# JunkyByte/deepcharuco

Measured on AMD Instinct MI355X. Metric: frames/sec end-to-end (detect+refine) at 320x240; corner-id match vs ref, higher is better.
Workload: dtype f32; 1 GPU; bs=32/GPU x1 GPU(s) = 32 frames of 320x240, full detect+refine pipeline (BASELINE configs[1]); preset=cfg2, batch_per_gpu=32, global_batch=32, height=240, width=320, corner_pool_per_gpu=2048, frames=board, truncated_frames=0, distinct_ids_in_batch=16, parallelism=frames sharded, 1 process/GPU x1

## Files before the change

deepcharuco_amd/_lib.py:

```python
from __future__ import annotations

import ctypes as C
import os
import subprocess
from typing import Optional

_HERE = os.path.dirname(os.path.abspath(__file__))
LIB_PATH = os.environ.get("DCX_LIB") or os.path.join(_HERE, "libdeepcharuco_amd.so")
CSRC = os.path.join(_HERE, "csrc")

_lib: Optional[C.CDLL] = None


class DcxError(RuntimeError):
    def __init__(self, code: int, where: str):
        self.code = code
        try:
            msg = lib().dcx_error_string(code).decode()
        except Exception:
            msg = "?"
        super().__init__(f"{where} failed with code {code}: {msg}")


def build(force: bool = False, verbose: bool = False) -> str:
# ... 3 lines not shown
    res = subprocess.run(cmd, capture_output=True, text=True)
    if res.returncode != 0:
        raise RuntimeError("building libdeepcharuco_amd.so failed:\n" + res.stdout[-4000:] + res.stderr[-8000:])
    if verbose:
        print(res.stdout)
    return LIB_PATH


_vp, _i, _l, _sz = C.c_void_p, C.c_int, C.c_long, C.c_size_t

SIGNATURES = {
    "dcx_version": (C.c_char_p, []),
    "dcx_error_string": (C.c_char_p, [_i]),
    "dcx_detector_create": (_i, [C.POINTER(_vp), C.POINTER(_vp), _i, _i]),
    "dcx_detector_destroy": (_i, [_vp]),
    "dcx_refiner_create": (_i, [C.POINTER(_vp), C.POINTER(_vp), _i]),
    "dcx_refiner_destroy": (_i, [_vp]),
    "dcx_detector_workspace_bytes": (_sz, [_vp, _i, _i, _i]),
    "dcx_refiner_workspace_bytes": (_sz, [_vp, _i]),
    "dcx_bgr2gray": (_i, [_vp, _l, _i, _i, _i, _i, _vp, _vp]),
    "dcx_bgr2gray_legacy14": (_i, [_vp, _l, _i, _i, _i, _i, _vp, _vp]),
    "dcx_pre_image": (_i, [_vp, _vp, _sz, _vp]),
    "dcx_detector_forward": (_i, [_vp, _vp, _l, _i, _vp, _i, _i, _i, _vp, _sz, _vp, _vp, _vp]),
    "dcx_detector_decode": (_i, [_vp, _i, _i, _i, _vp, _i, _i, _vp, _vp, _vp, _vp, _vp]),
    "dcx_pred_to_keypoints": (_i, [_vp, _vp, _i, _i, _i, _i, _i, _i, _i, _vp, _vp, _vp, _vp, _vp]),
    "dcx_label_to_keypoints": (_i, [_vp, _vp, _i, _i, _i, _i, _i, _vp, _vp, _vp, _vp, _vp]),
    "dcx_build_patch_table": (_i, [_vp, _vp, _i, _i, _vp, _vp, _vp]),
    "dcx_extract_patches_u8": (_i, [_vp, _l, _i, _i, _i, _vp, _vp, _i, _vp, _vp]),
    "dcx_extract_patches_f32": (_i, [_vp, _i, _i, _vp, _vp, _i, _vp, _vp]),
    "dcx_refiner_forward": (_i, [_vp, _vp, _i, _vp, _vp, _vp, _sz, _vp, _vp, _vp, _vp]),
    "dcx_argmax2d": (_i, [_vp, _i, _i, _i, _vp, _vp]),
    "dcx_pipeline_workspace_bytes": (_sz, [_vp, _vp, _i, _i, _i, _i]),
    "dcx_infer_batch": (_i, [_vp, _vp, _vp, _l, _i, _i, _i, _i, _i, _i, _i, _vp, _sz, _vp, _vp, _vp, _vp, _vp, _vp]),
    "dcx_stream_synchronize": (_i, [_vp]),
    "dcx_solve_pnp_pool": (_i, [_vp, _vp, _vp, _vp, _i, _i, _i, _i, C.c_double, C.POINTER(C.c_double), C.POINTER(C.c_double), _i,
                               _vp, _vp, _vp]),
    "dcx_solve_pnp_ransac_workspace_bytes": (_sz, [_i, _i, _i]),
    "dcx_solve_pnp_ransac_pool": (_i, [_vp, _vp, _vp, _vp, _i, _i, _i, _i, C.c_double, C.POINTER(C.c_double), C.POINTER(C.c_double), _i,
                                      _i, C.c_double, _i, C.c_uint, _vp, _sz, _vp, _vp, _vp, _vp, _vp]),
    "dcx_calibrate_workspace_bytes": (_sz, [_i]),
    "dcx_calibrate_pool": (_i, [_vp, _vp, _vp, _vp, _i, _i, _i, _i, C.c_double, _i, _i, _vp, _sz, _vp, _vp,
                               C.POINTER(C.c_double), _vp]),
    "dcx_calibrate_ransac_workspace_bytes": (_sz, [_i, _i, _i]),
    "dcx_calibrate_ransac_pool": (_i, [_vp, _vp, _vp, _vp, _i, _i, _i, _i, C.c_double, _i, _i, _i, C.c_double, C.c_double, _i, _i,
                                      C.c_uint, _vp, _sz, _vp, _vp, _vp, _vp, C.POINTER(C.c_double), _vp]),
    "dcx_stereo_calibrate_workspace_bytes": (_sz, [_i, _i, _i]),
    "dcx_stereo_calibrate_pool": (_i, [_vp] * 10 + [_i, _i, _i, _i, _i, C.c_double, C.POINTER(C.c_double), C.POINTER(C.c_double), _i,
                                      C.POINTER(C.c_double), C.POINTER(C.c_double), _i, _vp, _sz, _vp, _vp, _vp,
                                      C.POINTER(C.c_double), _vp]),
    "dcx_undistort_rectify_map": (_i, [C.POINTER(C.c_double), C.POINTER(C.c_double), _i, C.POINTER(C.c_double),
                                      C.POINTER(C.c_double), _i, _i, _vp, _vp]),
    "dcx_rectify_points_pool": (_i, [_vp, _vp, _i, C.POINTER(C.c_double), C.POINTER(C.c_double), _i, C.POINTER(C.c_double),
                                    C.POINTER(C.c_double), _vp, _vp]),
    "dcx_remap_u8": (_i, [_vp, _l, _i, _i, _i, _i, _vp, _i, _i, _i, _i, _vp, _vp]),
    "dcx_sgm_workspace_bytes": (_sz, [_i, _i, _i, _i]),
    "dcx_sgm_u8": (_i, [_vp, _l, _i, _vp, _l, _i, _i, _i, _i, _i, _i, _i, _i, _i, _i, _vp, _vp, _sz, _vp]),
    "dcx_sgm_u8_paths": (_i, [_vp, _l, _i, _vp, _l, _i, _i, _i, _i, _i, _i, _i, _i, _i, _i, _i, _vp, _vp, _sz, _vp]),
    "dcx_disparity_to_points": (_i, [_vp, _i, _i, _i, _i, C.POINTER(C.c_double), _vp, _vp]),
    "dcx_filter_speckles_workspace_bytes": (_sz, [_i, _i, _i]),
    "dcx_filter_speckles_s16": (_i, [_vp, _vp, _i, _i, _i, _i, _i, _i, _vp, _sz, _vp]),
    "dcx_conv_layer": (_i, [_vp, _i, _i, _i, _i, _vp, _vp, _vp, _vp, _vp, _vp, _i, _i, _i, _i, _i, _i, _vp, _vp]),
    "dcx_nchw_to_c4": (_i, [_vp, _i, _i, _i, _i, _vp, _vp]),
    "dcx_c4_to_nchw": (_i, [_vp, _i, _i, _i, _i, _vp, _vp]),
    "dcx_set_timing": (_i, [_i]),
    "dcx_get_timing": (_i, []),
    "dcx_profile_enabled": (_i, []),
# ... 63 lines not shown
```

deepcharuco_amd/csrc/dcx_api.hip:

```cpp
#include "dcx_common.h"

#include <math.h>
#include <stdlib.h>
#include <string.h>
#include <new>
#include <vector>

namespace {

constexpr float kBnEps = 1e-5f;

inline size_t align_up(size_t v, size_t a) { return (v + a - 1) / a * a; }


std::vector<float> pack_conv(const float* w, int cout, int cin, int ks, int cout_pad) {
    const int taps = ks * ks, cq = cin / 4;
    std::vector<float> out((size_t)taps * cq * cout_pad * 4, 0.0f);
    for (int o = 0; o < cout; ++o)
        for (int i = 0; i < cin; ++i)
            for (int t = 0; t < taps; ++t)
                out[(((size_t)t * cq + (i >> 2)) * cout_pad + o) * 4 + (i & 3)] = w[((size_t)o * cin + i) * taps + t];
    return out;
}

// ... 269 lines not shown
        std::vector<float> w(2 * wsz), b(512), g(512), be(512), mu(512), var(512);
        memcpy(w.data(), pa.w, wsz * 4); memcpy(w.data() + wsz, da.w, wsz * 4);
        auto cat = [](std::vector<float>& dst, const float* x, const float* y) {
            memcpy(dst.data(), x, 256 * 4); memcpy(dst.data() + 256, y, 256 * 4);
        };
        cat(b, pa.b, da.b); cat(g, pa.g, da.g); cat(be, pa.be, da.be); cat(mu, pa.mu, da.mu); cat(var, pa.var, da.var);
        rc = make_layer(HostConv{w.data(), b.data(), g.data(), be.data(), mu.data(), var.data()}, 128, 512, 3,
                        &d->heads_a);
    }
    if (rc == 0) rc = make_layer(hc(54, false), 256, 65, 1, &d->head_loc);
    if (rc == 0) rc = make_layer(hc(62, false), 256, n_ids + 1, 1, &d->head_ids);
    if (rc != 0) { dcx_detector_destroy(d); return rc; }
    *out = d;
    return 0;
}

extern "C" int dcx_detector_destroy(dcx_detector* d) {
    if (!d) return 0;
    free_layer(d->first);
    for (auto& l : d->enc) free_layer(l);
    free_layer(d->heads_a); free_layer(d->head_loc); free_layer(d->head_ids);
    delete d;
    return 0;
}

extern "C" size_t dcx_detector_workspace_bytes(const dcx_detector* det, int batch, int height, int width) {
    if (!det || batch <= 0 || height <= 0 || width <= 0) return 0;
    return det_layout(det->n_ids, batch, height, width).total;
}

namespace {
int detector_run(const dcx_detector* det, const uint8_t* d_frames_u8, long frame_stride, int pitch, int pix,
                 const float* d_images_f32, int batch, int height, int width, void* d_ws, size_t ws_bytes,
                 bool with_heads, float* d_loc_nchw, float* d_ids_nchw, int32_t* zero_words, int n_zero, void* stream);
}

extern "C" int dcx_detector_forward(const dcx_detector* det, const uint8_t* d_frames_u8, long frame_stride, int pitch,
                                    const float* d_images_f32, int batch, int height, int width, void* d_ws,
                                    size_t ws_bytes, float* d_loc_nchw, float* d_ids_nchw, void* stream) {
    return detector_run(det, d_frames_u8, frame_stride, pitch, DCX_PIX_GRAY8, d_images_f32, batch, height, width, d_ws, ws_bytes, true,
                        d_loc_nchw, d_ids_nchw, nullptr, 0, stream);
}

namespace {
int detector_run(const dcx_detector* det, const uint8_t* d_frames_u8, long frame_stride, int pitch, int pix,
                 const float* d_images_f32, int batch, int height, int width, void* d_ws, size_t ws_bytes,
                 bool with_heads, float* d_loc_nchw, float* d_ids_nchw, int32_t* zero_words, int n_zero, void* stream) {
    if (!det || !d_ws) return DCX_E_ARG;
    if ((d_frames_u8 == nullptr) == (d_images_f32 == nullptr)) return DCX_E_ARG;
    if (batch <= 0 || height < 8 || width < 8) return DCX_E_SHAPE;
    const DetWs L = det_layout(det->n_ids, batch, height, width);
    if (ws_bytes < L.total) return DCX_E_WS;
    hipStream_t s = (hipStream_t)stream;
    char* ws = (char*)d_ws;
    float* buf0 = (float*)(ws + L.buf0);
    float* buf1 = (float*)(ws + L.buf1);
    float* loc = (float*)(ws + L.loc);
    float* ids = (float*)(ws + L.ids);
    const int h = height, w = width;
    int rc;
    const int pt0 = dcx_prof_begin(DCX_PROF_CONV1A, batch, s);
    if (d_frames_u8)
        rc = dcx_launch_conv1_u8(d_frames_u8, frame_stride, pitch, pix, batch, h, w, 1, det->first.w, det->first.bias,
                                 det->first.alpha, det->first.beta, buf0, nullptr, zero_words, n_zero, s);
    else
        rc = dcx_launch_conv1_f32(d_images_f32, (long)h * w, w, batch, h, w, 1, det->first.w, det->first.bias,
                                  det->first.alpha, det->first.beta, buf0, nullptr, s);
    if (rc) return rc;
    if ((rc = dcx_prof_end(pt0, s))) return rc;
    struct Step { int layer, div, pool; };
    static const Step steps[7] = {{0, 1, 1}, {1, 2, 0}, {2, 2, 1}, {3, 4, 0}, {4, 4, 1}, {5, 8, 0}, {6, 8, 0}};
    float* src = buf0;
    float* dst = buf1;
    for (const Step& st : steps) {
        const DevLayer& l = det->enc[st.layer];
        DcxConvArgs a = conv_args(l, src, batch, l.cin / 4, 0, h / st.div, w / st.div, 0, 1, dst, l.cout / 4, nullptr);
        rc = dcx_launch_conv_mfma(a, 3, st.pool, DCX_EPI_BNRELU, s);
        if (rc) return rc;
        float* t = src; src = dst; dst = t;
    }
    const int hc = h / 8, wc = w / 8;
    {
        DcxConvArgs a = conv_args(det->heads_a, src, batch, 32, 0, hc, wc, 0, 1, dst, 128, nullptr);
        rc = dcx_launch_conv_mfma(a, 3, 0, DCX_EPI_BNRELU, s);
        if (rc) return rc;
    }
    if (!with_heads) return 0;
    {
        DcxConvArgs a = conv_args(det->head_loc, dst, batch, 128, 0, 1, hc * wc, 0, 0, loc, 17, nullptr);
        rc = dcx_launch_conv_mfma(a, 1, 0, DCX_EPI_RAW, s);
        if (rc) return rc;
    }
    {
        DcxConvArgs a = conv_args(det->head_ids, dst, batch, 128, 64, 1, hc * wc, 0, 0, ids, L.ids_quads, nullptr);
        rc = dcx_launch_conv_mfma(a, 1, 0, DCX_EPI_RAW, s);
        if (rc) return rc;
    }
    if (d_loc_nchw) { rc = dcx_c4_to_nchw(loc, batch, 65, hc, wc, d_loc_nchw, stream); if (rc) return rc; }
    if (d_ids_nchw) { rc = dcx_c4_to_nchw(ids, batch, det->n_ids + 1, hc, wc, d_ids_nchw, stream); if (rc) return rc; }
    return 0;
}
}

extern "C" int dcx_detector_decode(const dcx_detector* det, int batch, int height, int width, void* d_ws,
                                   int dust_bin, int kmax, int32_t* d_counts, int32_t* d_rows, int32_t* d_loc_argmax,
                                   int32_t* d_ids_argmax, void* stream) {
    if (!det || !d_ws) return DCX_E_ARG;
    if (batch <= 0 || height < 8 || width < 8) return DCX_E_SHAPE;
    const DetWs L = det_layout(det->n_ids, batch, height, width);
    const int hc = height / 8, wc = width / 8;
    const long cells = (long)hc * wc;
    char* ws = (char*)d_ws;
// ... 91 lines not shown
        {7, 16, 1, 1, 0},
        {8, 32, 0, 1, 0},
    };
    float* src = buf0;
    float* dst = buf1;
    for (const Step& st : steps) {
        const DevLayer& l = rf->mid[st.layer];
        DcxConvArgs a = conv_args(l, src, p, l.cin / 4, 0, st.hin, st.hin, st.ups, st.pad, dst, l.cout / 4, lim);
        a.n_hint = lim != nullptr ? n_hint : 0;
        rc = dcx_launch_conv_mfma(a, 3, st.pool, DCX_EPI_BNRELU, s);
        if (rc) return rc;
        float* t = src; src = dst; dst = t;
    }
    int heat_tiles = 0;
    {
        DcxConvArgs a = conv_args(rf->head_a, src, p, 16, 0, 32, 32, 1, 1, nullptr, 16, lim);
        a.head_w = rf->head_w; a.head_b = rf->head_b; a.heat = d_heat;
        a.part_val = (float*)(ws + L.pval); a.part_idx = (int*)(ws + L.pidx);
        heat_tiles = dcx_conv_heat_tiles(a.ho, a.wo, a.w_ups2w != nullptr ? 1 : 0);
        if (heat_tiles <= 0 || heat_tiles > kRefTiles) return DCX_E_SHAPE;
        rc = dcx_launch_conv_mfma(a, 3, 0, DCX_EPI_HEAT, s);
        if (rc) return rc;
    }
    const int pt1 = dcx_prof_begin(DCX_PROF_FINALIZE, p, s);
    rc = dcx_launch_refine_finalize((const float*)(ws + L.pval), (const int*)(ws + L.pidx), heat_tiles, 64, p, lim,
                                    d_table, d_corners, d_xy, s);
    if (rc) return rc;
    return dcx_prof_end(pt1, s);
}
}

namespace {
struct PipeWs { size_t det, table, ctrl, ref, total; int ctrl_words; };
PipeWs pipe_layout(const dcx_detector* det, const dcx_refiner* rf, int b, int h, int w, int pool) {
    PipeWs L;
    size_t off = 0;
    L.det = off; off = align_up(off + det_layout(det->n_ids, b, h, w).total, 256);
    L.table = off; off = align_up(off + (size_t)pool * 16, 256);
    L.ctrl_words = 64 + b;
    L.ctrl = off; off = align_up(off + (size_t)L.ctrl_words * 4, 256);
    L.ref = off; off = align_up(off + (rf ? ref_layout(pool).total : 0), 256);
    L.total = off;
    return L;
}
}

extern "C" size_t dcx_pipeline_workspace_bytes(const dcx_detector* det, const dcx_refiner* rf, int batch, int height,
                                               int width, int pool) {
    if (!det || batch <= 0 || height <= 0 || width <= 0 || pool <= 0) return 0;
    return pipe_layout(det, rf, batch, height, width, pool).total;
}

namespace {
int infer_range(const dcx_detector* det, const dcx_refiner* rf, const uint8_t* d_frames_u8, long frame_stride, int pitch, int pix,
                int batch, int height, int width, int dust_bin, int pool, char* ws, size_t ws_bytes, int32_t* d_counts,
                int32_t* d_starts, int32_t* d_rows, float* d_xy, float* d_conf, hipStream_t s, bool timing) {
    void* stream = (void*)s;
    const PipeWs L = pipe_layout(det, rf, batch, height, width, pool);
    if (ws_bytes < L.total) return DCX_E_WS;
    int rc = timing ? timing_mark(0, s) : 0;
    if (rc) return rc;
    int32_t* ctrl = (int32_t*)(ws + L.ctrl);
    rc = detector_run(det, d_frames_u8, frame_stride, pitch, pix, nullptr, batch, height, width, ws + L.det, L.table - L.det,
                      false, nullptr, nullptr, ctrl, L.ctrl_words, stream);
    if (rc) return rc;
    if (timing && (rc = timing_mark(1, s))) return rc;
    int32_t* table = (int32_t*)(ws + L.table);
    {
        const DetWs D = det_layout(det->n_ids, batch, height, width);
        const int hc = height / 8, wc = width / 8;
        const float* act = (const float*)(ws + L.det + D.buf0);
        int32_t* codes = (int32_t*)(ws + L.det + D.codes);
        DcxPoolOut po;
        po.tickets = ctrl + 64; po.cursor = ctrl; po.counts = d_counts; po.starts = d_starts; po.rows = d_rows;
        po.table = rf ? table : nullptr; po.conf = d_conf; po.conf_cells = (float*)(ws + L.det + D.conf);
        po.wc = wc; po.pool = pool;
        const int pt = dcx_prof_begin(DCX_PROF_TAIL, batch, s);
        rc = dcx_launch_tail(act, batch, hc * wc, det->head_loc.w, det->head_loc.bias, det->head_ids.w, det->head_ids.bias,
                             det->head_ids.cout_pad, det->n_ids + 1, dust_bin, codes, nullptr, nullptr, &po, s);
        if (rc) return rc;
        if ((rc = dcx_prof_end(pt, s))) return rc;
    }
    if (timing && (rc = timing_mark(2, s))) return rc;
    if (rf == nullptr) return timing ? timing_mark(3, s) : 0;
    const long expect = (long)batch * det->n_ids;
    const FrameSrc src{d_frames_u8, frame_stride, pitch, pix, height, width};
    rc = refiner_run(rf, nullptr, &src, pool, (int)(expect < pool ? expect : pool), ctrl, table,
                     ws + L.ref, L.total - L.ref, nullptr, d_xy, nullptr, stream);
    if (rc) return rc;
    return timing ? timing_mark(3, s) : 0;
}
}

extern "C" int dcx_infer_batch(const dcx_detector* det, const dcx_refiner* rf, const uint8_t* d_frames_u8,
                               long frame_stride, int pitch, int pixel_format, int batch, int height, int width, int dust_bin,
                               int pool, void* d_ws, size_t ws_bytes, int32_t* d_counts, int32_t* d_starts, int32_t* d_rows,
                               float* d_xy, float* d_conf, void* stream) {
    if (!det || !d_frames_u8 || !d_ws || !d_counts || !d_starts || !d_rows) return DCX_E_ARG;
    if (rf != nullptr && d_xy == nullptr) return DCX_E_ARG;
    if (pixel_format != DCX_PIX_GRAY8 && pixel_format != DCX_PIX_BGR8 && pixel_format != DCX_PIX_BGR8_LEGACY14) return DCX_E_ARG;
    if (pool <= 0 || pool > (1 << 22)) return DCX_E_SHAPE;
    if (batch <= 0 || batch > (1 << 20) || height < 8 || width < 8) return DCX_E_SHAPE;
    if (pitch < width * (pixel_format == DCX_PIX_GRAY8 ? 1 : 3)) return DCX_E_SHAPE;
    if (dust_bin < 0 || dust_bin > 255) return DCX_E_NIDS;
    hipStream_t s = (hipStream_t)stream;
    char* ws = (char*)d_ws;
    return infer_range(det, rf, d_frames_u8, frame_stride, pitch, pixel_format, batch, height, width, dust_bin, pool, ws, ws_bytes,
                       d_counts, d_starts, d_rows, d_xy, d_conf, s, true);
}

extern "C" int dcx_stream_synchronize(void* stream) { return (int)hipStreamSynchronize((hipStream_t)stream); }

extern "C" int dcx_set_timing(int enabled) { g_timing = enabled != 0; return 0; }
extern "C" int dcx_get_timing(void) { return g_timing ? 1 : 0; }

extern "C" int dcx_last_timings(float* h_ms4) {
    if (!h_ms4) return DCX_E_ARG;
    if (!g_ev_ok) return DCX_E_ARG;
    DCX_CHECK_HIP(hipEventElapsedTime(&h_ms4[0], g_ev[0], g_ev[1]));
    DCX_CHECK_HIP(hipEventElapsedTime(&h_ms4[1], g_ev[1], g_ev[2]));
    DCX_CHECK_HIP(hipEventElapsedTime(&h_ms4[2], g_ev[2], g_ev[3]));
    DCX_CHECK_HIP(hipEventElapsedTime(&h_ms4[3], g_ev[0], g_ev[3]));
    return 0;
}

extern "C" int dcx_conv_layer(const float* d_in, int n, int cin, int hin, int win, const float* h_w, const float* h_b,
                              const float* h_g, const float* h_be, const float* h_mu, const float* h_var, int cout,
                              int ksize, int pad, int ups, int pool, int relu, float* d_out, void* stream) {
    if (!d_in || !h_w || !h_b || !d_out) return DCX_E_ARG;
    if (cin % 32 != 0 || (ksize != 3 && ksize != 1) || n <= 0) return DCX_E_SHAPE;
    const bool bn = h_g != nullptr;
    if (bn != (relu != 0)) return DCX_E_ARG;
    if (bn && (!h_be || !h_mu || !h_var)) return DCX_E_ARG;
    if (const int rc = dcx_xcd_init()) return rc;
    DevLayer l;
    int rc = make_layer(HostConv{h_w, h_b, h_g, h_be, h_mu, h_var}, cin, cout, ksize, &l, ups != 0);
    if (rc) return rc;
    DcxConvArgs a;
    if (ksize == 1) {
        if (pad != 0 || ups != 0 || pool != 0) { free_layer(l); return DCX_E_SHAPE; }
        a = conv_args(l, d_in, n, cin / 4, 0, 1, hin * win, 0, 0, d_out, (cout + 3) / 4, nullptr);
// ... 10 lines not shown
```

deepcharuco_amd/inference.py:

```python
from __future__ import annotations

import ctypes as _ctypes
import warnings
from typing import List, Optional

import numpy as np
import torch

from . import _lib
from .imgproc import _opencv, bgr2gray
from .models._handles import require_cuda, unwrap
from .models.model_utils import extract_patches, pre_bgr_image, pred_to_keypoints
from .models.net import dcModel, lModel
from .models.refinenet import RefineNet, lRefineNet
from .pnp import (solve_pnp_batch_device, solve_pnp_device, solve_pnp_host, solve_pnp_pool, solve_pnp_ransac_batch_device,
                  solve_pnp_ransac_device, solve_pnp_ransac_host, solve_pnp_ransac_pool, unpack_poses, unpack_ransac)

__all__ = ["load_models", "infer_image", "infer_image_staged", "infer_batch", "infer_batch_device", "unpack_results", "packed_len",
           "solve_pnp", "solve_pnp_batch", "solve_pnp_submit", "set_deterministic", "InferenceModel", "calibrate_xcd",
           "set_xcd_weights", "get_xcd_weights", "solve_pnp_host", "solve_pnp_device", "solve_pnp_batch_device", "solve_pnp_pool",
           "unpack_poses", "solve_pnp_ransac_host", "solve_pnp_ransac_device", "solve_pnp_ransac_batch_device",
           "solve_pnp_ransac_pool", "unpack_ransac"]

DEFAULT_KMAX = 64
# ... 83 lines not shown
    with torch.cuda.device(dev):
        torch.cuda.synchronize()
        _lib.check(_lib.lib().dcx_calibrate_xcd(int(rounds), w, _lib.current_stream()), "dcx_calibrate_xcd")
    from .graph import clear_graph_cache
    clear_graph_cache()
    return [float(v) for v in w]


def set_xcd_weights(weights=None, device="cuda") -> None:
    dev = require_cuda(device)
    arr = None if weights is None else (_ctypes.c_float * 8)(*[float(v) for v in weights])
    with torch.cuda.device(dev):
        _lib.check(_lib.lib().dcx_set_xcd_weights(arr), "dcx_set_xcd_weights")
    from .graph import clear_graph_cache
    clear_graph_cache()


def get_xcd_weights(device="cuda") -> List[float]:
    dev = require_cuda(device)
    w = (_ctypes.c_float * 8)()
    with torch.cuda.device(dev):
        _lib.check(_lib.lib().dcx_get_xcd_weights(w), "dcx_get_xcd_weights")
    return [float(v) for v in w]


PIXEL_FORMATS = {"gray": 0, "opencv4": 1, "legacy14": 2}


def packed_len(batch: int, pool: int, conf: bool = False) -> int:
    return 2 * batch + (8 if conf else 6) * pool


def launch_pipeline(det, ref, frames_ptr: int, b: int, h: int, w: int, bpp: int, pix: int, dust_bin_ids: int, pool: int,
                    ws: torch.Tensor, out_ptr: int, conf: bool = False) -> None:
    counts_p, starts_p, rows_p = out_ptr, out_ptr + 4 * b, out_ptr + 8 * b
    xy_p = rows_p + 16 * pool
    conf_p = xy_p + 8 * pool
    _lib.check(_lib.lib().dcx_infer_batch(det.handle, ref.handle if ref else None, frames_ptr, h * w * bpp, w * bpp, pix, b, h, w,
                                          dust_bin_ids, pool, ws.data_ptr(), ws.numel(), counts_p, starts_p, rows_p,
                                          xy_p if ref else None, conf_p if conf else None, _lib.current_stream()), "dcx_infer_batch")


def infer_batch_device(frames: torch.Tensor, dust_bin_ids: int, deepc, refinenet=None, kmax: int = DEFAULT_KMAX,
                       out: Optional[torch.Tensor] = None, ws: Optional[torch.Tensor] = None, pool: Optional[int] = None,
                       conf: bool = False, bgr_variant: str = "opencv4") -> torch.Tensor:
    det, ref = unwrap(deepc), unwrap(refinenet)
    dev = det.device
    if (not isinstance(frames, torch.Tensor) or frames.device != dev or frames.dtype != torch.uint8 or not frames.is_contiguous()
            or not (frames.ndim == 3 or (frames.ndim == 4 and frames.shape[3] == 3))):
        raise ValueError("frames must be a contiguous (B,H,W) gray or (B,H,W,3) BGR uint8 tensor on the model's GPU")
    b, h, w = frames.shape[:3]
    bpp = 1 if frames.ndim == 3 else 3
    if bgr_variant not in ("opencv4", "legacy14"):
        raise ValueError(f"unknown BGR->gray variant {bgr_variant!r}")
    pix = PIXEL_FORMATS["gray" if bpp == 1 else bgr_variant]
    if pool is None:
        pool = b * kmax
    if pool <= 0:
        raise ValueError("pool must be positive")
    L = _lib.lib()
    with torch.cuda.device(dev):
        nbytes = L.dcx_pipeline_workspace_bytes(det.handle, ref.handle if ref else None, b, h, w, pool)
        if nbytes == 0:
            raise ValueError("bad batch/shape for dcx_pipeline_workspace_bytes")
        if ws is None:
            ws = det._ws.get("pipe", dev, nbytes)
        elif ws.device != dev or ws.dtype != torch.uint8 or not ws.is_contiguous() or ws.numel() < nbytes:
            raise ValueError(f"ws must be a contiguous uint8 tensor of >= {nbytes} bytes on {dev}")
        n_i32 = packed_len(b, pool, conf)
        if out is None:
            out = torch.empty((n_i32,), dtype=torch.int32, device=dev)
        elif out.device != dev or out.dtype != torch.int32 or out.numel() != n_i32 or not out.is_contiguous():
            raise ValueError(f"out must be a contiguous int32 tensor of {n_i32} elements on {dev}")
        launch_pipeline(det, ref, frames.data_ptr(), b, h, w, bpp, pix, dust_bin_ids, pool, ws, out.data_ptr(), conf)
    return out


def unpack_results(packed: np.ndarray, batch: int, pool: int, refined: bool, conf: bool = False):
    packed = np.asarray(packed, dtype=np.int32)
    counts = packed[:batch]
    head = packed[:2 * batch].tolist()
    rows = packed[2 * batch:2 * batch + 4 * pool].reshape(pool, 4)
    xy = packed[2 * batch + 4 * pool:2 * batch + 6 * pool].view(np.float32).reshape(pool, 2)
    cf = packed[2 * batch + 6 * pool:2 * batch + 8 * pool].view(np.float32).reshape(pool, 2) if conf else None
    res: List[Optional[np.ndarray]] = []
    confs: List[Optional[np.ndarray]] = []
    for b in range(batch):
        k, s0 = head[b], head[batch + b]
        if k == 0:
            res.append(np.array([]))
            confs.append(np.zeros((0, 2), np.float32))
            continue
        if s0 + k > pool:
            res.append(None)
            confs.append(None)
            continue
        rb = rows[s0:s0 + k]
        order = rb[:, 2].argsort(kind="stable")
        a = np.empty((k, 3), np.float64 if refined else np.int64)
        a[:, 0:2] = xy[s0:s0 + k] if refined else rb[:, 0:2]
        a[:, 2] = rb[:, 2]
# ... 143 lines not shown
```

deepcharuco_amd/stream.py:

```python
from __future__ import annotations

import time
import warnings
from typing import Iterable, Iterator, List, Optional, Tuple

import numpy as np
import torch

from .inference import DEFAULT_KMAX, infer_batch, infer_batch_device, packed_len, solve_pnp_submit, unpack_results
from .models._handles import unwrap
from .pnp import (POSE_WORDS, ransac_workspace_bytes, solve_pnp_batch_device, solve_pnp_pool, solve_pnp_ransac_batch_device,
                  solve_pnp_ransac_pool, unpack_poses, unpack_ransac)


class FrameStream:
    def __init__(self, dust_bin_ids: int, deepc, refinenet=None, batch: int = 32, height: int = 240,
                 width: int = 320, kmax: int = DEFAULT_KMAX, depth: int = 2, pnp: Optional[dict] = None,
                 compute_streams: int = 1, bgr: bool = False, h2d_on_compute: Optional[bool] = None, pnp_device: bool = False,
                 pnp_ransac: Optional[dict] = None):
        det = unwrap(deepc)
        self.dev = det.device
        self.dust_bin_ids, self.deepc, self.refinenet = dust_bin_ids, deepc, refinenet
        self.batch, self.h, self.w, self.kmax, self.depth = batch, height, width, kmax, depth
        self.pool = batch * kmax
        self.bgr = bool(bgr)
        self.h2d_on_compute = compute_streams > 1 if h2d_on_compute is None else bool(h2d_on_compute)
        self.pnp = pnp
        self.pnp_device = bool(pnp_device) and pnp is not None
        if pnp_ransac is not None and not self.pnp_device:
            raise ValueError("pnp_ransac needs pnp=... and pnp_device=True")
        self.pnp_ransac = None if pnp_ransac is None else dict(pnp_ransac)
        if not (1 <= compute_streams <= depth):
            raise ValueError("compute_streams must be between 1 and depth")
        n_out = packed_len(batch, self.pool)
        shape = (batch, height, width, 3) if self.bgr else (batch, height, width)
        with torch.cuda.device(self.dev):
            self.copy_stream = torch.cuda.Stream()
            self.compute = [torch.cuda.Stream() for _ in range(compute_streams)] if compute_streams > 1 else None
            self.pin_in = [torch.empty(shape, dtype=torch.uint8).pin_memory() for _ in range(depth)]
            self.dev_in = [torch.empty(shape, dtype=torch.uint8, device=self.dev) for _ in range(depth)]
            self.dev_out = [torch.empty((n_out,), dtype=torch.int32, device=self.dev) for _ in range(depth)]
            self.pin_out = [torch.empty((n_out,), dtype=torch.int32).pin_memory() for _ in range(depth)]
# ... 84 lines not shown
        return retired

    def _resolve(self, r):
        return r if len(r) == 2 or self.pnp_device else (r[0], r[1], [f.result() for f in r[2]])

    def flush(self) -> Iterator[Tuple]:
        order = sorted((p[0], s) for s, p in enumerate(self._pending) if p is not None)
        for _, slot in order:
            yield self._resolve(self._collect(slot))

    def run(self, batches: Iterable[np.ndarray]) -> Iterator[Tuple]:
        if self.pnp is None:
            for fr in batches:
                r = self.submit(fr)
                if r is not None:
                    yield r
            yield from self.flush()
            return
        held = None
        for fr in batches:
            r = self.submit(fr)
            if held is not None:
                yield self._resolve(held)
                held = None
            if r is not None:
                held = r
        if held is not None:
            yield self._resolve(held)
        yield from self.flush()


class ResidentStream:

    def __init__(self, dust_bin_ids: int, deepc, refinenet=None, batch: int = 32, height: int = 240, width: int = 320,
                 kmax: int = DEFAULT_KMAX, compute_streams: int = 1, depth: Optional[int] = None, bgr: bool = False,
                 raw: bool = False, timing: bool = False):
        det = unwrap(deepc)
        self.dev = det.device
        self.dust_bin_ids, self.deepc, self.refinenet = dust_bin_ids, deepc, refinenet
        self.batch, self.h, self.w, self.kmax = batch, height, width, kmax
        self.pool = batch * kmax
        self.bgr, self.raw, self.timing = bool(bgr), bool(raw), bool(timing)
        if compute_streams < 1:
            raise ValueError("compute_streams must be >= 1")
        self.depth = depth = compute_streams + 2 if depth is None else depth
        if depth < compute_streams:
            raise ValueError("depth must be >= compute_streams")
        n_out = packed_len(batch, self.pool)
        with torch.cuda.device(self.dev):
            self.compute = [torch.cuda.Stream() for _ in range(compute_streams)]
            self.dev_out = [torch.empty((n_out,), dtype=torch.int32, device=self.dev) for _ in range(depth)]
            self.pin_out = [torch.empty((n_out,), dtype=torch.int32).pin_memory() for _ in range(depth)]
            self.ev_in = [torch.cuda.Event() for _ in range(depth)]
            self.ev_start = [torch.cuda.Event(enable_timing=True) for _ in range(depth)] if self.timing else None
            self.ev_done = [torch.cuda.Event(enable_timing=self.timing) for _ in range(depth)]
        self._pending: List[Optional[Tuple[int, torch.Tensor, torch.cuda.Stream]]] = [None] * depth
        self._ticket = 0
        self.gpu_ms: List[float] = []
        self.host_enqueue_s = 0.0
        self.host_wait_s = 0.0

    def reset_stats(self) -> None:
        self.gpu_ms = []
        self.host_enqueue_s = self.host_wait_s = 0.0

    def _collect(self, slot: int):
        ticket, frames, compute = self._pending[slot]
        self._pending[slot] = None
        n = frames.shape[0]
        t0 = time.perf_counter()
        self.ev_done[slot].synchronize()
        self.host_wait_s += time.perf_counter() - t0
        if self.timing:
            self.gpu_ms.append(self.ev_start[slot].elapsed_time(self.ev_done[slot]))
        packed = self.pin_out[slot].numpy()[:packed_len(n, self.pool)]
        need = int(packed[:n].astype(np.int64).sum())
        if need > self.pool:
            warnings.warn(f"a batch produced {need} corners > pool={self.pool} (batch x kmax); re-running it with pool={need}")
            n_big = packed_len(n, need)
            with torch.cuda.device(self.dev):
                host = torch.empty((n_big,), dtype=torch.int32).pin_memory()
                done = torch.cuda.Event()
                with torch.cuda.stream(compute):
                    big = infer_batch_device(frames, self.dust_bin_ids, self.deepc, self.refinenet, pool=need)
                    host.copy_(big, non_blocking=True)
                    done.record(compute)
            t0 = time.perf_counter()
            done.synchronize()
            self.host_wait_s += time.perf_counter() - t0
            packed = host.numpy()
            if self.raw:
                return ticket, packed
            return ticket, unpack_results(packed, n, need, self.refinenet is not None)[0]
        if self.raw:
            return ticket, packed.copy()
        return ticket, unpack_results(packed, n, self.pool, self.refinenet is not None)[0]

    def submit(self, frames: torch.Tensor):
        want = (self.h, self.w, 3) if self.bgr else (self.h, self.w)
        if (not isinstance(frames, torch.Tensor) or frames.device != self.dev or frames.dtype != torch.uint8
                or not frames.is_contiguous() or tuple(frames.shape[1:]) != want or not (1 <= frames.shape[0] <= self.batch)):
            raise ValueError(f"frames must be a contiguous (1 <= n <= batch, {', '.join(map(str, want))}) uint8 tensor on {self.dev}")
        n = frames.shape[0]
        slot = self._ticket % self.depth
        retired = self._collect(slot) if self._pending[slot] is not None else None
        t0 = time.perf_counter()
        n_out = packed_len(n, self.pool)
        with torch.cuda.device(self.dev):
            compute = self.compute[self._ticket % len(self.compute)]
            self.ev_in[slot].record(torch.cuda.current_stream())
            with torch.cuda.stream(compute):
                compute.wait_event(self.ev_in[slot])
                if self.timing:
                    self.ev_start[slot].record(compute)
                infer_batch_device(frames, self.dust_bin_ids, self.deepc, self.refinenet, out=self.dev_out[slot][:n_out],
                                   pool=self.pool)
                self.pin_out[slot][:n_out].copy_(self.dev_out[slot][:n_out], non_blocking=True)
                self.ev_done[slot].record(compute)
        self._pending[slot] = (self._ticket, frames, compute)
        self._ticket += 1
        self.host_enqueue_s += time.perf_counter() - t0
        return retired

    def flush(self) -> Iterator[Tuple]:
        order = sorted((p[0], s) for s, p in enumerate(self._pending) if p is not None)
        for _, slot in order:
            yield self._collect(slot)

    def run(self, batches: Iterable[torch.Tensor]) -> Iterator[Tuple]:
        for fr in batches:
            r = self.submit(fr)
            if r is not None:
                yield r
        yield from self.flush()
```

include/deepcharuco_amd.h:

```cpp
#ifndef DEEPCHARUCO_AMD_H
#define DEEPCHARUCO_AMD_H

#include <stddef.h>
#include <stdint.h>

#ifdef __cplusplus
extern "C" {
#endif

#define DCX_E_ARG      (-1)
#define DCX_E_SHAPE    (-2)
#define DCX_E_WS       (-3)
#define DCX_E_NIDS     (-4)

typedef struct dcx_detector dcx_detector;
typedef struct dcx_refiner  dcx_refiner;

const char* dcx_version(void);
const char* dcx_error_string(int code);

int dcx_detector_create(dcx_detector** out, const float* const* h_tensors, int n_tensors, int n_ids);
int dcx_detector_destroy(dcx_detector* det);
int dcx_refiner_create(dcx_refiner** out, const float* const* h_tensors, int n_tensors);
int dcx_refiner_destroy(dcx_refiner* rf);
// ... 24 lines not shown
                          int dust_bin, int kmax,
                          int32_t* d_counts, int32_t* d_rows,
                          int32_t* d_loc_argmax, int32_t* d_ids_argmax, void* stream);
int dcx_label_to_keypoints(const long long* d_loc, const long long* d_ids, int batch, int hc, int wc, int dust_bin, int kmax,
                           int32_t* d_counts, int32_t* d_rows, int32_t* d_codes, int32_t* d_bad, void* stream);

int dcx_build_patch_table(const int32_t* d_counts, const int32_t* d_rows, int batch, int kmax,
                          int32_t* d_table, int32_t* d_total, void* stream);

int dcx_extract_patches_u8(const uint8_t* d_frames, long frame_stride, int pitch, int height, int width,
                           const int32_t* d_table, const int32_t* d_total, int max_patches,
                           float* d_patches, void* stream);
int dcx_extract_patches_f32(const float* d_images, int height, int width,
                            const int32_t* d_table, const int32_t* d_total, int max_patches,
                            float* d_patches, void* stream);

int dcx_refiner_forward(const dcx_refiner* rf, const float* d_patches, int max_patches,
                        const int32_t* d_total, const int32_t* d_table,
                        void* d_ws, size_t ws_bytes,
                        int32_t* d_corners, float* d_xy, float* d_heat, void* stream);

int dcx_argmax2d(const float* d_x, int k, int h, int w, int32_t* d_out, void* stream);

#define DCX_PIX_GRAY8          0
#define DCX_PIX_BGR8           1
#define DCX_PIX_BGR8_LEGACY14  2
size_t dcx_pipeline_workspace_bytes(const dcx_detector* det, const dcx_refiner* rf,
                                    int batch, int height, int width, int pool);
int dcx_infer_batch(const dcx_detector* det, const dcx_refiner* rf,
                    const uint8_t* d_frames_u8, long frame_stride, int pitch, int pixel_format,
                    int batch, int height, int width, int dust_bin, int pool,
                    void* d_ws, size_t ws_bytes,
                    int32_t* d_counts, int32_t* d_starts, int32_t* d_rows, float* d_xy, float* d_conf, void* stream);
int dcx_stream_synchronize(void* stream);

#define DCX_PNP_OK          0
#define DCX_PNP_TOO_FEW     1
#define DCX_PNP_TRUNCATED   2
#define DCX_PNP_BAD_ID      3
#define DCX_PNP_DEGENERATE  4
#define DCX_PNP_NONFINITE   5
int dcx_solve_pnp_pool(const int32_t* d_counts, const int32_t* d_starts, const int32_t* d_rows,
                       const float* d_xy , int batch, int pool,
                       int col_count, int row_count, double square_len,
                       const double* h_camera9, const double* h_dist, int n_dist,
                       int32_t* d_status, double* d_pose ,
                       void* stream);

#define DCX_PNP_NO_CONSENSUS 6
size_t dcx_solve_pnp_ransac_workspace_bytes(int batch, int pool, int iterations);
int dcx_solve_pnp_ransac_pool(const int32_t* d_counts, const int32_t* d_starts, const int32_t* d_rows,
                              const float* d_xy , int batch, int pool,
                              int col_count, int row_count, double square_len,
                              const double* h_camera9, const double* h_dist, int n_dist,
                              int iterations, double reproj_error, int min_inliers, unsigned seed,
                              void* d_workspace, size_t workspace_bytes,
                              int32_t* d_status, double* d_pose , int32_t* d_info ,
                              uint8_t* d_inliers , void* stream);

#define DCX_CALIB_OK          0
#define DCX_CALIB_NO_VIEWS    1
#define DCX_CALIB_DEGENERATE  2
#define DCX_CALIB_NONFINITE   3
size_t dcx_calibrate_workspace_bytes(int batch);
int dcx_calibrate_pool(const int32_t* d_counts, const int32_t* d_starts, const int32_t* d_rows,
                       const float* d_xy , int batch, int pool,
// ... 98 lines not shown
```

Before: 10240 frames/s.

## Prefetch conv1a on a side stream to overlap with previous batch's tail

Splits the first detector conv (conv1a from u8 frames) into a separate entry point that writes into a double-buffered front workspace on a side stream. The main compute stream waits on that event and runs the rest of the pipeline from the prefetched activation, recording a detector-done event so the next front launch can reuse the buffer safely. This lets conv1a of batch N+1 overlap with decode/refine of batch N. The pipeline also now writes results straight into pinned host memory, dropping the device output buffer and the device-to-host copy. The cost is two extra full-resolution 64-channel activation buffers plus the added cross-stream event synchronisation.

```diff
diff --git a/deepcharuco_amd/_lib.py b/deepcharuco_amd/_lib.py
--- a/deepcharuco_amd/_lib.py
+++ b/deepcharuco_amd/_lib.py
@@ -59,6 +59,10 @@
     "dcx_argmax2d": (_i, [_vp, _i, _i, _i, _vp, _vp]),
     "dcx_pipeline_workspace_bytes": (_sz, [_vp, _vp, _i, _i, _i, _i]),
     "dcx_infer_batch": (_i, [_vp, _vp, _vp, _l, _i, _i, _i, _i, _i, _i, _i, _vp, _sz, _vp, _vp, _vp, _vp, _vp, _vp]),
+    "dcx_front_bytes": (_sz, [_vp, _i, _i, _i]),
+    "dcx_detector_front": (_i, [_vp, _vp, _l, _i, _i, _i, _i, _i, _vp, _sz, _vp]),
+    "dcx_infer_batch_prefetched": (_i, [_vp, _vp, _vp, _l, _i, _i, _i, _i, _i, _i, _i, _vp, _sz, _vp, _sz, _vp, _vp, _vp, _vp, _vp,
+                                       _vp, _vp]),
     "dcx_stream_synchronize": (_i, [_vp]),
     "dcx_solve_pnp_pool": (_i, [_vp, _vp, _vp, _vp, _i, _i, _i, _i, C.c_double, C.POINTER(C.c_double), C.POINTER(C.c_double), _i,
                                _vp, _vp, _vp]),
diff --git a/deepcharuco_amd/csrc/dcx_api.hip b/deepcharuco_amd/csrc/dcx_api.hip
--- a/deepcharuco_amd/csrc/dcx_api.hip
+++ b/deepcharuco_amd/csrc/dcx_api.hip
@@ -325,20 +325,36 @@
 namespace {
 int detector_run(const dcx_detector* det, const uint8_t* d_frames_u8, long frame_stride, int pitch, int pix,
                  const float* d_images_f32, int batch, int height, int width, void* d_ws, size_t ws_bytes,
-                 bool with_heads, float* d_loc_nchw, float* d_ids_nchw, int32_t* zero_words, int n_zero, void* stream);
+                 bool with_heads, float* d_loc_nchw, float* d_ids_nchw, int32_t* zero_words, int n_zero, const float* act0,
+                 void* stream);
 }
 
 extern "C" int dcx_detector_forward(const dcx_detector* det, const uint8_t* d_frames_u8, long frame_stride, int pitch,
                                     const float* d_images_f32, int batch, int height, int width, void* d_ws,
                                     size_t ws_bytes, float* d_loc_nchw, float* d_ids_nchw, void* stream) {
     return detector_run(det, d_frames_u8, frame_stride, pitch, DCX_PIX_GRAY8, d_images_f32, batch, height, width, d_ws, ws_bytes, true,
-                        d_loc_nchw, d_ids_nchw, nullptr, 0, stream);
-}
-
-namespace {
+                        d_loc_nchw, d_ids_nchw, nullptr, 0, nullptr, stream);
+}
+
+namespace {
+int detector_front(const dcx_detector* det, const uint8_t* d_frames_u8, long frame_stride, int pitch, int pix,
+                   const float* d_images_f32, int batch, int h, int w, float* out, int32_t* zero_words, int n_zero, hipStream_t s) {
+    int rc;
+    const int pt0 = dcx_prof_begin(DCX_PROF_CONV1A, batch, s);
+    if (d_frames_u8)
+        rc = dcx_launch_conv1_u8(d_frames_u8, frame_stride, pitch, pix, batch, h, w, 1, det->first.w, det->first.bias,
+                                 det->first.alpha, det->first.beta, out, nullptr, zero_words, n_zero, s);
+    else
+        rc = dcx_launch_conv1_f32(d_images_f32, (long)h * w, w, batch, h, w, 1, det->first.w, det->first.bias,
+                                  det->first.alpha, det->first.beta, out, nullptr, s);
+    if (rc) return rc;
+    return dcx_prof_end(pt0, s);
+}
+
 int detector_run(const dcx_detector* det, const uint8_t* d_frames_u8, long frame_stride, int pitch, int pix,
                  const float* d_images_f32, int batch, int height, int width, void* d_ws, size_t ws_bytes,
-                 bool with_heads, float* d_loc_nchw, float* d_ids_nchw, int32_t* zero_words, int n_zero, void* stream) {
+                 bool with_heads, float* d_loc_nchw, float* d_ids_nchw, int32_t* zero_words, int n_zero, const float* act0,
+                 void* stream) {
     if (!det || !d_ws) return DCX_E_ARG;
     if ((d_frames_u8 == nullptr) == (d_images_f32 == nullptr)) return DCX_E_ARG;
     if (batch <= 0 || height < 8 || width < 8) return DCX_E_SHAPE;
@@ -352,25 +368,19 @@
     float* ids = (float*)(ws + L.ids);
     const int h = height, w = width;
     int rc;
-    const int pt0 = dcx_prof_begin(DCX_PROF_CONV1A, batch, s);
-    if (d_frames_u8)
-        rc = dcx_launch_conv1_u8(d_frames_u8, frame_stride, pitch, pix, batch, h, w, 1, det->first.w, det->first.bias,
-                                 det->first.alpha, det->first.beta, buf0, nullptr, zero_words, n_zero, s);
-    else
-        rc = dcx_launch_conv1_f32(d_images_f32, (long)h * w, w, batch, h, w, 1, det->first.w, det->first.bias,
-                                  det->first.alpha, det->first.beta, buf0, nullptr, s);
-    if (rc) return rc;
-    if ((rc = dcx_prof_end(pt0, s))) return rc;
+    if (act0 == nullptr && (rc = detector_front(det, d_frames_u8, frame_stride, pitch, pix, d_images_f32, batch, h, w, buf0,
+                                                zero_words, n_zero, s)))
+        return rc;
     struct Step { int layer, div, pool; };
     static const Step steps[7] = {{0, 1, 1}, {1, 2, 0}, {2, 2, 1}, {3, 4, 0}, {4, 4, 1}, {5, 8, 0}, {6, 8, 0}};
-    float* src = buf0;
+    const float* src = act0 ? act0 : buf0;
     float* dst = buf1;
     for (const Step& st : steps) {
         const DevLayer& l = det->enc[st.layer];
         DcxConvArgs a = conv_args(l, src, batch, l.cin / 4, 0, h / st.div, w / st.div, 0, 1, dst, l.cout / 4, nullptr);
         rc = dcx_launch_conv_mfma(a, 3, st.pool, DCX_EPI_BNRELU, s);
         if (rc) return rc;
-        float* t = src; src = dst; dst = t;
+        src = dst; dst = dst == buf1 ? buf0 : buf1;
     }
     const int hc = h / 8, wc = w / 8;
     {
@@ -528,12 +538,23 @@
 
 namespace {
 struct PipeWs { size_t det, table, ctrl, ref, total; int ctrl_words; };
+inline int ctrl_word_count(int b) { return 64 + b; }
+struct FrontWs { size_t act, ctrl, total; int ctrl_words; };
+FrontWs front_layout(int b, int h, int w) {
+    FrontWs F;
+    size_t off = 0;
+    F.act = off; off = align_up(off + (size_t)b * 64 * h * w * 4, 256);
+    F.ctrl_words = ctrl_word_count(b);
+    F.ctrl = off; off = align_up(off + (size_t)F.ctrl_words * 4, 256);
+    F.total = off;
+    return F;
+}
 PipeWs pipe_layout(const dcx_detector* det, const dcx_refiner* rf, int b, int h, int w, int pool) {
     PipeWs L;
     size_t off = 0;
     L.det = off; off = align_up(off + det_layout(det->n_ids, b, h, w).total, 256);
     L.table = off; off = align_up(off + (size_t)pool * 16, 256);
-    L.ctrl_words = 64 + b;
+    L.ctrl_words = ctrl_word_count(b);
     L.ctrl = off; off = align_up(off + (size_t)L.ctrl_words * 4, 256);
     L.ref = off; off = align_up(off + (rf ? ref_layout(pool).total : 0), 256);
     L.total = off;
@@ -547,19 +568,50 @@
     return pipe_layout(det, rf, batch, height, width, pool).total;
 }
 
+extern "C" size_t dcx_front_bytes(const dcx_detector* det, int batch, int height, int width) {
+    if (!det || batch <= 0 || height <= 0 || width <= 0) return 0;
+    return front_layout(batch, height, width).total;
+}
+
+namespace {
+int check_batch_args(const dcx_detector* det, const uint8_t* d_frames_u8, int pitch, int pixel_format, int batch, int height,
+                     int width) {
+    if (!det || !d_frames_u8) return DCX_E_ARG;
+    if (pixel_format != DCX_PIX_GRAY8 && pixel_format != DCX_PIX_BGR8 && pixel_format != DCX_PIX_BGR8_LEGACY14) return DCX_E_ARG;
+    if (batch <= 0 || batch > (1 << 20) || height < 8 || width < 8) return DCX_E_SHAPE;
+    if (pitch < width * (pixel_format == DCX_PIX_GRAY8 ? 1 : 3)) return DCX_E_SHAPE;
+    return 0;
+}
+}
+
+extern "C" int dcx_detector_front(const dcx_detector* det, const uint8_t* d_frames_u8, long frame_stride, int pitch,
+                                  int pixel_format, int batch, int height, int width, void* d_front, size_t front_bytes,
+                                  void* stream) {
+    if (!d_front) return DCX_E_ARG;
+    if (const int rc = check_batch_args(det, d_frames_u8, pitch, pixel_format, batch, height, width)) return rc;
+    const FrontWs F = front_layout(batch, height, width);
+    if (front_bytes < F.total) return DCX_E_WS;
+    char* front = (char*)d_front;
+    return detector_front(det, d_frames_u8, frame_stride, pitch, pixel_format, nullptr, batch, height, width, (float*)(front + F.act),
+                          (int32_t*)(front + F.ctrl), F.ctrl_words, (hipStream_t)stream);
+}
+
 namespace {
 int infer_range(const dcx_detector* det, const dcx_refiner* rf, const uint8_t* d_frames_u8, long frame_stride, int pitch, int pix,
-                int batch, int height, int width, int dust_bin, int pool, char* ws, size_t ws_bytes, int32_t* d_counts,
-                int32_t* d_starts, int32_t* d_rows, float* d_xy, float* d_conf, hipStream_t s, bool timing) {
+                int batch, int height, int width, int dust_bin, int pool, char* ws, size_t ws_bytes, char* front,
+                hipEvent_t detector_done, int32_t* d_counts, int32_t* d_starts, int32_t* d_rows, float* d_xy, float* d_conf,
+                hipStream_t s, bool timing) {
     void* stream = (void*)s;
     const PipeWs L = pipe_layout(det, rf, batch, height, width, pool);
     if (ws_bytes < L.total) return DCX_E_WS;
     int rc = timing ? timing_mark(0, s) : 0;
     if (rc) return rc;
-    int32_t* ctrl = (int32_t*)(ws + L.ctrl);
+    const FrontWs F = front_layout(batch, height, width);
+    int32_t* ctrl = (int32_t*)(front ? front + F.ctrl : ws + L.ctrl);
     rc = detector_run(det, d_frames_u8, frame_stride, pitch, pix, nullptr, batch, height, width, ws + L.det, L.table - L.det,
-                      false, nullptr, nullptr, ctrl, L.ctrl_words, stream);
+                      false, nullptr, nullptr, ctrl, L.ctrl_words, front ? (const float*)(front + F.act) : nullptr, stream);
     if (rc) return rc;
+    if (detector_done) DCX_CHECK_HIP(hipEventRecord(detector_done, s));
     if (timing && (rc = timing_mark(1, s))) return rc;
     int32_t* table = (int32_t*)(ws + L.table);
     {
@@ -602,7 +654,23 @@
     hipStream_t s = (hipStream_t)stream;
     char* ws = (char*)d_ws;
     return infer_range(det, rf, d_frames_u8, frame_stride, pitch, pixel_format, batch, height, width, dust_bin, pool, ws, ws_bytes,
-                       d_counts, d_starts, d_rows, d_xy, d_conf, s, true);
+                       nullptr, nullptr, d_counts, d_starts, d_rows, d_xy, d_conf, s, true);
+}
+
+extern "C" int dcx_infer_batch_prefetched(const dcx_detector* det, const dcx_refiner* rf, const uint8_t* d_frames_u8,
+                                          long frame_stride, int pitch, int pixel_format, int batch, int height, int width,
+                                          int dust_bin, int pool, void* d_ws, size_t ws_bytes, void* d_front, size_t front_bytes,
+                                          int32_t* d_counts, int32_t* d_starts, int32_t* d_rows, float* d_xy, float* d_conf,
+                                          void* detector_done_event, void* stream) {
+    if (!d_ws || !d_front || !d_counts || !d_starts || !d_rows) return DCX_E_ARG;
+    if (rf != nullptr && d_xy == nullptr) return DCX_E_ARG;
+    if (const int rc = check_batch_args(det, d_frames_u8, pitch, pixel_format, batch, height, width)) return rc;
+    if (pool <= 0 || pool > (1 << 22)) return DCX_E_SHAPE;
+    if (dust_bin < 0 || dust_bin > 255) return DCX_E_NIDS;
+    if (front_bytes < front_layout(batch, height, width).total) return DCX_E_WS;
+    return infer_range(det, rf, d_frames_u8, frame_stride, pitch, pixel_format, batch, height, width, dust_bin, pool, (char*)d_ws,
+                       ws_bytes, (char*)d_front, (hipEvent_t)detector_done_event, d_counts, d_starts, d_rows, d_xy, d_conf,
+                       (hipStream_t)stream, true);
 }
 
 extern "C" int dcx_stream_synchronize(void* stream) { return (int)hipStreamSynchronize((hipStream_t)stream); }
diff --git a/deepcharuco_amd/inference.py b/deepcharuco_amd/inference.py
--- a/deepcharuco_amd/inference.py
+++ b/deepcharuco_amd/inference.py
@@ -139,13 +139,36 @@
 
 
 def launch_pipeline(det, ref, frames_ptr: int, b: int, h: int, w: int, bpp: int, pix: int, dust_bin_ids: int, pool: int,
-                    ws: torch.Tensor, out_ptr: int, conf: bool = False) -> None:
+                    ws: torch.Tensor, out_ptr: int, conf: bool = False, front: Optional[torch.Tensor] = None,
+                    detector_done: Optional[int] = None) -> None:
     counts_p, starts_p, rows_p = out_ptr, out_ptr + 4 * b, out_ptr + 8 * b
     xy_p = rows_p + 16 * pool
     conf_p = xy_p + 8 * pool
-    _lib.check(_lib.lib().dcx_infer_batch(det.handle, ref.handle if ref else None, frames_ptr, h * w * bpp, w * bpp, pix, b, h, w,
-                                          dust_bin_ids, pool, ws.data_ptr(), ws.numel(), counts_p, starts_p, rows_p,
-                                          xy_p if ref else None, conf_p if conf else None, _lib.current_stream()), "dcx_infer_batch")
+    head = (det.handle, ref.handle if ref else None, frames_ptr, h * w * bpp, w * bpp, pix, b, h, w, dust_bin_ids, pool,
+            ws.data_ptr(), ws.numel())
+    tail = (counts_p, starts_p, rows_p, xy_p if ref else None, conf_p if conf else None, _lib.current_stream())
+    if front is None:
+        _lib.check(_lib.lib().dcx_infer_batch(*head, *tail), "dcx_infer_batch")
+    else:
+        _lib.check(_lib.lib().dcx_infer_batch_prefetched(*head, front.data_ptr(), front.numel(), *tail[:-1], detector_done, tail[-1]),
+                   "dcx_infer_batch_prefetched")
+
+
+def launch_front(det, frames_ptr: int, b: int, h: int, w: int, bpp: int, pix: int, front: torch.Tensor) -> None:
+    _lib.check(_lib.lib().dcx_detector_front(det.handle, frames_ptr, h * w * bpp, w * bpp, pix, b, h, w, front.data_ptr(),
+                                             front.numel(), _lib.current_stream()), "dcx_detector_front")
+
+
+def pipeline_workspace(det, ref, b: int, h: int, w: int, pool: int, ws: Optional[torch.Tensor] = None) -> torch.Tensor:
+    dev = det.device
+    nbytes = _lib.lib().dcx_pipeline_workspace_bytes(det.handle, ref.handle if ref else None, b, h, w, pool)
+    if nbytes == 0:
+        raise ValueError("bad batch/shape for dcx_pipeline_workspace_bytes")
+    if ws is None:
+        return det._ws.get("pipe", dev, nbytes)
+    if ws.device != dev or ws.dtype != torch.uint8 or not ws.is_contiguous() or ws.numel() < nbytes:
+        raise ValueError(f"ws must be a contiguous uint8 tensor of >= {nbytes} bytes on {dev}")
+    return ws
 
 
 def infer_batch_device(frames: torch.Tensor, dust_bin_ids: int, deepc, refinenet=None, kmax: int = DEFAULT_KMAX,
@@ -165,15 +188,8 @@
         pool = b * kmax
     if pool <= 0:
         raise ValueError("pool must be positive")
-    L = _lib.lib()
     with torch.cuda.device(dev):
-        nbytes = L.dcx_pipeline_workspace_bytes(det.handle, ref.handle if ref else None, b, h, w, pool)
-        if nbytes == 0:
-            raise ValueError("bad batch/shape for dcx_pipeline_workspace_bytes")
-        if ws is None:
-            ws = det._ws.get("pipe", dev, nbytes)
-        elif ws.device != dev or ws.dtype != torch.uint8 or not ws.is_contiguous() or ws.numel() < nbytes:
-            raise ValueError(f"ws must be a contiguous uint8 tensor of >= {nbytes} bytes on {dev}")
+        ws = pipeline_workspace(det, ref, b, h, w, pool, ws)
         n_i32 = packed_len(b, pool, conf)
         if out is None:
             out = torch.empty((n_i32,), dtype=torch.int32, device=dev)
diff --git a/deepcharuco_amd/stream.py b/deepcharuco_amd/stream.py
--- a/deepcharuco_amd/stream.py
+++ b/deepcharuco_amd/stream.py
@@ -1,5 +1,6 @@
 from __future__ import annotations
 
+import os
 import time
 import warnings
 from typing import Iterable, Iterator, List, Optional, Tuple
@@ -7,7 +8,9 @@
 import numpy as np
 import torch
 
-from .inference import DEFAULT_KMAX, infer_batch, infer_batch_device, packed_len, solve_pnp_submit, unpack_results
+from . import _lib
+from .inference import (DEFAULT_KMAX, PIXEL_FORMATS, infer_batch, infer_batch_device, launch_front, launch_pipeline, packed_len, pipeline_workspace, solve_pnp_submit,
+                        unpack_results)
 from .models._handles import unwrap
 from .pnp import (POSE_WORDS, ransac_workspace_bytes, solve_pnp_batch_device, solve_pnp_pool, solve_pnp_ransac_batch_device,
                   solve_pnp_ransac_pool, unpack_poses, unpack_ransac)
@@ -158,9 +161,11 @@
 
 class ResidentStream:
 
+    PREFETCH_MAX_BYTES = 1 << 30
+
     def __init__(self, dust_bin_ids: int, deepc, refinenet=None, batch: int = 32, height: int = 240, width: int = 320,
                  kmax: int = DEFAULT_KMAX, compute_streams: int = 1, depth: Optional[int] = None, bgr: bool = False,
-                 raw: bool = False, timing: bool = False):
+                 raw: bool = False, timing: bool = False, prefetch: Optional[bool] = None):
         det = unwrap(deepc)
         self.dev = det.device
         self.dust_bin_ids, self.deepc, self.refinenet = dust_bin_ids, deepc, refinenet
@@ -175,11 +180,32 @@
         n_out = packed_len(batch, self.pool)
         with torch.cuda.device(self.dev):
             self.compute = [torch.cuda.Stream() for _ in range(compute_streams)]
-            self.dev_out = [torch.empty((n_out,), dtype=torch.int32, device=self.dev) for _ in range(depth)]
             self.pin_out = [torch.empty((n_out,), dtype=torch.int32).pin_memory() for _ in range(depth)]
             self.ev_in = [torch.cuda.Event() for _ in range(depth)]
             self.ev_start = [torch.cuda.Event(enable_timing=True) for _ in range(depth)] if self.timing else None
             self.ev_done = [torch.cuda.Event(enable_timing=self.timing) for _ in range(depth)]
+            self._front = None
+            if prefetch and compute_streams != 1:
+                raise ValueError("prefetch needs compute_streams == 1 (several streams already overlap everything)")
+            nb = _lib.lib().dcx_front_bytes(det.handle, batch, height, width)
+            if prefetch is None and os.environ.get("DCX_RS_PREFETCH"):
+                prefetch = os.environ["DCX_RS_PREFETCH"] != "0"
+            if os.environ.get("DCX_RS_PRIO", "0") != "0":
+                self.compute = [torch.cuda.Stream(priority=-1)]
+            if prefetch is None:
+                prefetch = compute_streams == 1 and nb <= self.PREFETCH_MAX_BYTES
+            if prefetch and compute_streams == 1:
+                try:
+                    self._front = [torch.empty((nb,), dtype=torch.uint8, device=self.dev) for _ in range(2)]
+                except torch.cuda.OutOfMemoryError:
+                    warnings.warn(f"ResidentStream: no memory for two prefetch sets of {nb} bytes; running without the conv1a prefetch")
+                else:
+                    self.side = torch.cuda.Stream()
+                    self.ev_front = [torch.cuda.Event() for _ in range(depth)]
+                    self.ev_det = [torch.cuda.Event() for _ in range(depth)]
+                    for e in self.ev_det:
+                        e.record(self.side)
+                    self._last_det: Optional[torch.cuda.Event] = None
         self._pending: List[Optional[Tuple[int, torch.Tensor, torch.cuda.Stream]]] = [None] * depth
         self._ticket = 0
         self.gpu_ms: List[float] = []
@@ -231,17 +257,30 @@
         slot = self._ticket % self.depth
         retired = self._collect(slot) if self._pending[slot] is not None else None
         t0 = time.perf_counter()
-        n_out = packed_len(n, self.pool)
         with torch.cuda.device(self.dev):
             compute = self.compute[self._ticket % len(self.compute)]
             self.ev_in[slot].record(torch.cuda.current_stream())
+            det, ref = unwrap(self.deepc), unwrap(self.refinenet)
+            bpp, pix = (3, PIXEL_FORMATS["opencv4"]) if self.bgr else (1, PIXEL_FORMATS["gray"])
+            front = None
+            if self._front is not None:
+                front = self._front[self._ticket % 2]
+                with torch.cuda.stream(self.side):
+                    self.side.wait_event(self.ev_in[slot])
+                    if self._last_det is not None:
+                        self.side.wait_event(self._last_det)
+                    launch_front(det, frames.data_ptr(), n, self.h, self.w, bpp, pix, front)
+                    self.ev_front[slot].record(self.side)
+                self._last_det = self.ev_det[slot]
             with torch.cuda.stream(compute):
                 compute.wait_event(self.ev_in[slot])
                 if self.timing:
                     self.ev_start[slot].record(compute)
-                infer_batch_device(frames, self.dust_bin_ids, self.deepc, self.refinenet, out=self.dev_out[slot][:n_out],
-                                   pool=self.pool)
-                self.pin_out[slot][:n_out].copy_(self.dev_out[slot][:n_out], non_blocking=True)
+                if front is not None:
+                    compute.wait_event(self.ev_front[slot])
+                launch_pipeline(det, ref, frames.data_ptr(), n, self.h, self.w, bpp, pix, self.dust_bin_ids, self.pool,
+                                pipeline_workspace(det, ref, n, self.h, self.w, self.pool), self.pin_out[slot].data_ptr(), front=front,
+                                detector_done=self.ev_det[slot].cuda_event if front is not None else None)
                 self.ev_done[slot].record(compute)
         self._pending[slot] = (self._ticket, frames, compute)
         self._ticket += 1
diff --git a/include/deepcharuco_amd.h b/include/deepcharuco_amd.h
--- a/include/deepcharuco_amd.h
+++ b/include/deepcharuco_amd.h
@@ -80,6 +80,15 @@
                     int batch, int height, int width, int dust_bin, int pool,
                     void* d_ws, size_t ws_bytes,
                     int32_t* d_counts, int32_t* d_starts, int32_t* d_rows, float* d_xy, float* d_conf, void* stream);
+size_t dcx_front_bytes(const dcx_detector* det, int batch, int height, int width);
+int dcx_detector_front(const dcx_detector* det, const uint8_t* d_frames_u8, long frame_stride, int pitch, int pixel_format,
+                       int batch, int height, int width, void* d_front, size_t front_bytes, void* stream);
+int dcx_infer_batch_prefetched(const dcx_detector* det, const dcx_refiner* rf,
+                               const uint8_t* d_frames_u8, long frame_stride, int pitch, int pixel_format,
+                               int batch, int height, int width, int dust_bin, int pool,
+                               void* d_ws, size_t ws_bytes, void* d_front, size_t front_bytes,
+                               int32_t* d_counts, int32_t* d_starts, int32_t* d_rows, float* d_xy, float* d_conf,
+                               void* detector_done_event, void* stream);
 int dcx_stream_synchronize(void* stream);
 
 #define DCX_PNP_OK          0
```

Measured after the change: 10410 frames/s, median of 6. +1.6%, better.
